# bjack205/LQR.jl

Measured on NVIDIA B200. Metric: batched LQR KKT solves/sec (FP64), higher is better.
Workload: dtype f64

## Files before the change

### lqr.jl_b200/csrc/riccati.cu

```cuda
#include <algorithm>
#include <cstdio>

#include "riccati_kernels.cuh"
#include "riccati_dmma_kernels.cuh"
#include "riccati_cta_kernels.cuh"

#define RICCATI_TPI_SIZES(X) \
    X(2, 1) X(3, 2) X(4, 1) X(4, 2) X(6, 3) X(2, 2) X(3, 1) X(3, 3) X(4, 3) X(5, 1) X(5, 2) X(5, 3) X(6, 1) X(6, 2)

static bool riccati_has_tpi(int n, int m) {
#define X(N_, M_) \
    if (n == N_ && m == M_) return true;
    RICCATI_TPI_SIZES(X)
#undef X
    return false;
}

#define RICCATI_DMMA_SIZES(X) X(8, 1) X(8, 2) X(8, 3) X(8, 4) X(12, 1) X(12, 2) X(12, 3) X(12, 4)

static bool riccati_has_dmma(int n, int m) {
#define X(N_, M_) \
    if (n == N_ && m == M_) return true;
    RICCATI_DMMA_SIZES(X)
#undef X
    return false;
}

#define RICCATI_CTA_SIZES(X) X(16, 8) X(16, 16) X(24, 8) X(24, 16) X(32, 8) X(32, 16) X(48, 16) X(64, 16)

static bool riccati_has_cta(int n, int m) {
#define X(N_, M_) \
    if (n == N_ && m == M_) return true;
    RICCATI_CTA_SIZES(X)
#undef X
    return false;
}

int lqrb_riccati_tile(const lqrb_context *h, int n, int m) {
    const int64_t force = h->opt("riccati_variant", 0);
    if (force == 2) return 1;
    return riccati_has_tpi(n, m) ? LQRB_TILE : 1;
}

static std::vector<RowMap> riccati_knot_map(int n, int m, int N, int flags) {
    const int Kn = (flags & LQRB_FLAG_LTI) ? 1 : N - 1;
    std::vector<RowMap> map;
    map.reserve((size_t)Kn * (n * n + n * m + tri(n) + tri(m) + n + m));
    for (int k = 0; k < Kn; ++k) {
        for (int e = 0; e < n * n; ++e) map.push_back({0, k * n * n + e, 0.0});
        for (int e = 0; e < n * m; ++e) map.push_back({1, k * n * m + e, 0.0});
        for (int j = 0; j < n; ++j)
            for (int i = 0; i <= j; ++i) map.push_back({2, k * n * n + i + j * n, 0.0});
        for (int j = 0; j < m; ++j)
            for (int i = 0; i <= j; ++i) map.push_back({3, k * m * m + i + j * m, 0.0});
        for (int e = 0; e < n; ++e) map.push_back({4, k * n + e, 0.0});
        for (int e = 0; e < m; ++e) map.push_back({5, k * m + e, 0.0});
        if (lqrb_riccati_knot_rows(n, m) > n * n + n * m + tri(n) + tri(m) + n + m) map.push_back({-1, 0, 0.0});
    }
    return map;
}

static std::vector<RowMap> riccati_term_map(int n) {
    std::vector<RowMap> map;
    for (int j = 0; j < n; ++j)
        for (int i = 0; i <= j; ++i) map.push_back({6, i + j * n, 0.0});
    for (int e = 0; e < n; ++e) map.push_back({7, e, 0.0});
    for (int e = 0; e < n; ++e) map.push_back({8, e, 0.0});
    return map;
}

static std::vector<RowMap> riccati_gain_map(int n, int m, int N) {
    std::vector<RowMap> map;
    for (int k = 0; k < N - 1; ++k) {
        for (int e = 0; e < m * n; ++e) map.push_back({0, k * m * n + e, 0.0});
        for (int e = 0; e < m; ++e) map.push_back({1, k * m + e, 0.0});
    }
    return map;
}

static std::string key(const char *tag, int a, int b, int c, int d) {
    char buf[96];
    snprintf(buf, sizeof buf, "%s:%d:%d:%d:%d", tag, a, b, c, d);
    return buf;
}

static int32_t check_dims(lqrb_context *h, int n, int m, int N, int64_t batch) {
    if (!h) return -1;
    if (n < 1 || n > 128) return lqrb_fail(h, -2, "n out of range [1,128]");
    if (m < 1 || m > n) return lqrb_fail(h, -3, "m out of range [1,n]");
    if (N < 2) return lqrb_fail(h, -4, "N must be >= 2");
    if (batch < 0) return lqrb_fail(h, -5, "batch must be >= 0");
    return 0;
}

template <int n, int m, bool LTI, int THREADS, int MINB>
static void launch_tpi_cfg(int N, int64_t batch, const double *knots, const double *term, double *Z,
                           double *gains, int32_t *info, cudaStream_t s) {
    const unsigned grid = (unsigned)((batch + THREADS - 1) / THREADS);
    riccati_tpi_kernel<n, m, LTI, THREADS, MINB><<<grid, THREADS, 0, s>>>(knots, term, Z, gains, info, N, batch);
}

template <int n, int m>
static int32_t launch_tpi(lqrb_context *h, int N, int64_t batch, int lti, const double *knots,
                          const double *term, double *Z, double *gains, int32_t *info,
                          cudaStream_t s) {
    constexpr bool SMALL = (n * n + n * m) <= 20;
    const bool tight = SMALL && h->opt("riccati_tpi_cfg", 0) != 1;
    if (SMALL && tight) {
        if (lti) launch_tpi_cfg<n, m, true, 64, 8>(N, batch, knots, term, Z, gains, info, s);
        else launch_tpi_cfg<n, m, false, 64, 8>(N, batch, knots, term, Z, gains, info, s);
    } else {
        if (lti) launch_tpi_cfg<n, m, true, 128, 1>(N, batch, knots, term, Z, gains, info, s);
        else launch_tpi_cfg<n, m, false, 128, 1>(N, batch, knots, term, Z, gains, info, s);
    }
    char nm[64];
    snprintf(nm, sizeof nm, "riccati_tpi<%d,%d>%s%s", n, m, lti ? "[lti]" : "", tight ? "[64x8]" : "[128x1]");
    h->kernel_name = nm;
    LQRB_LAUNCH_CHECK(h, "riccati_tpi_kernel");
    return 0;
}

static int32_t launch_coop(lqrb_context *h, int n, int m, int N, int64_t batch, int lti,
                           const double *knots, const double *term, double *Z, double *gains,
                           int32_t *info, cudaStream_t s) {
    const size_t per = riccati_coop_smem_doubles(n, m) * sizeof(double);
    char nm[64];
    if (n + m <= 24) {
        constexpr int G = 32, THREADS = 128;
        const size_t smem = per * (THREADS / G);
        auto kern = riccati_coop_kernel<G, THREADS>;
        LQRB_CUDA(h, cudaFuncSetAttribute(kern, cudaFuncAttributeMaxDynamicSharedMemorySize, (int)smem));
        const unsigned grid = (unsigned)((batch + THREADS / G - 1) / (THREADS / G));
        kern<<<grid, THREADS, smem, s>>>(knots, term, Z, gains, info, n, m, N, lti, batch);
        snprintf(nm, sizeof nm, "riccati_coop<G=32>(n=%d,m=%d)", n, m);
    } else {
        constexpr int G = 256, THREADS = 256;
        if (per > 227 * 1024) return lqrb_fail(h, -2, "n,m too large for the shared-memory Riccati kernel");
        auto kern = riccati_coop_kernel<G, THREADS>;
        LQRB_CUDA(h, cudaFuncSetAttribute(kern, cudaFuncAttributeMaxDynamicSharedMemorySize, (int)per));
        kern<<<(unsigned)batch, THREADS, per, s>>>(knots, term, Z, gains, info, n, m, N, lti, batch);
        snprintf(nm, sizeof nm, "riccati_coop<G=256>(n=%d,m=%d)", n, m);
    }
    h->kernel_name = nm;
    LQRB_LAUNCH_CHECK(h, "riccati_coop_kernel");
    return 0;
}

template <int n, int m>
static int32_t launch_dmma(lqrb_context *h, int N, int64_t batch, int lti, const double *knots,
                           const double *term, double *Z, double *gains, int32_t *info,
                           cudaStream_t s) {
    constexpr int STAGES = 3, WARPS = 4, MINB = m == 1 ? 6 : 5;
    const size_t smem = rdmma::riccati_dmma_warp_smem(rdmma::Map<n, m>::F, STAGES) * WARPS;
    auto kern = rdmma::riccati_dmma_kernel<n, m, STAGES, WARPS, MINB>;
    LQRB_CUDA(h, cudaFuncSetAttribute(kern, cudaFuncAttributeMaxDynamicSharedMemorySize, (int)smem));
    const unsigned grid = (unsigned)((batch + WARPS - 1) / WARPS);
    kern<<<grid, WARPS * 32, smem, s>>>(knots, term, Z, gains, info, N, lti, batch);
    char nm[64];
    snprintf(nm, sizeof nm, "riccati_dmma<%d,%d>%s", n, m, lti ? "[lti]" : "");
    h->kernel_name = nm;
    LQRB_LAUNCH_CHECK(h, "riccati_dmma_kernel");
    return 0;
}

template <int n, int m>
static int32_t launch_cta(lqrb_context *h, int N, int64_t batch, int lti, const double *knots,
                          const double *term, double *Z, double *gains, int32_t *info, cudaStream_t s) {
    using C = rcta::Cfg<n, m>;
    auto kern = rcta::riccati_cta_kernel<n, m>;
    LQRB_CUDA(h, cudaFuncSetAttribute(kern, cudaFuncAttributeMaxDynamicSharedMemorySize, (int)C::SMEM));
    kern<<<(unsigned)batch, C::THREADS, C::SMEM, s>>>(knots, term, Z, gains, info, N, lti, batch);
    char nm[64];
    snprintf(nm, sizeof nm, "riccati_cta_dmma<%d,%d>%s", n, m, lti ? "[lti]" : "");
    h->kernel_name = nm;
    LQRB_LAUNCH_CHECK(h, "riccati_cta_kernel");
    return 0;
}

static bool riccati_pad_target(const lqrb_context *h, int n, int m, int *n2, int *m2) {
    if (h->opt("riccati_pad", 1) == 0 || h->opt("riccati_variant", 0) != 0) return false;
    if (lqrb_riccati_tile(h, n, m) == LQRB_TILE || riccati_has_dmma(n, m) || riccati_has_cta(n, m)) return false;
#define X(N_, M_) \
    if (n <= N_ && m <= M_) { *n2 = N_; *m2 = M_; return true; }
    RICCATI_DMMA_SIZES(X)
    RICCATI_CTA_SIZES(X)
#undef X
    return false;
}

namespace {
struct RiccatiPadMaps {
    std::vector<RowMap> knots, term, z, gains;
};
}

static RiccatiPadMaps riccati_pad_maps(int n, int m, int N, int Kn, int n2, int m2) {
    RiccatiPadMaps M;
    const int F = lqrb_riccati_knot_rows(n, m), F2 = lqrb_riccati_knot_rows(n2, m2);
    const int nn = n * n, nm = n * m, tn = tri(n), tm = tri(m);
    for (int k = 0; k < Kn; ++k) {
        const int32_t b = k * F;
        const size_t start = M.knots.size();
        for (int j = 0; j < n2; ++j)
            for (int i = 0; i < n2; ++i) M.knots.push_back((i < n && j < n) ? RowMap{0, b + i + j * n, 0.0} : RowMap{-1, 0, 0.0});
        for (int j = 0; j < m2; ++j)
            for (int i = 0; i < n2; ++i)
                M.knots.push_back((i < n && j < m) ? RowMap{0, b + nn + i + j * n, 0.0} : RowMap{-1, 0, 0.0});
        for (int j = 0; j < n2; ++j)
            for (int i = 0; i <= j; ++i)
                M.knots.push_back(j < n ? RowMap{0, b + nn + nm + j * (j + 1) / 2 + i, 0.0} : RowMap{-1, 0, i == j ? 1.0 : 0.0});
        for (int j = 0; j < m2; ++j)
            for (int i = 0; i <= j; ++i)
                M.knots.push_back(j < m ? RowMap{0, b + nn + nm + tn + j * (j + 1) / 2 + i, 0.0} : RowMap{-1, 0, i == j ? 1.0 : 0.0});
        for (int i = 0; i < n2; ++i) M.knots.push_back(i < n ? RowMap{0, b + nn + nm + tn + tm + i, 0.0} : RowMap{-1, 0, 0.0});
        for (int i = 0; i < m2; ++i) M.knots.push_back(i < m ? RowMap{0, b + nn + nm + tn + tm + n + i, 0.0} : RowMap{-1, 0, 0.0});
        while (M.knots.size() - start < (size_t)F2) M.knots.push_back(RowMap{-1, 0, 0.0});
    }
    for (int j = 0; j < n2; ++j)
        for (int i = 0; i <= j; ++i) M.term.push_back(j < n ? RowMap{0, j * (j + 1) / 2 + i, 0.0} : RowMap{-1, 0, i == j ? 1.0 : 0.0});
    for (int i = 0; i < n2; ++i) M.term.push_back(i < n ? RowMap{0, tn + i, 0.0} : RowMap{-1, 0, 0.0});
    for (int i = 0; i < n2; ++i) M.term.push_back(i < n ? RowMap{0, tn + n + i, 0.0} : RowMap{-1, 0, 0.0});
    for (int k = 0; k < N; ++k) {
        for (int i = 0; i < n2; ++i) M.z.push_back(i < n ? RowMap{0, k * (n + m) + i, 0.0} : RowMap{-1, 0, 0.0});
        if (k < N - 1)
            for (int i = 0; i < m2; ++i) M.z.push_back(i < m ? RowMap{0, k * (n + m) + n + i, 0.0} : RowMap{-1, 0, 0.0});
    }
    const int GR = m * n + m;
    for (int k = 0; k < N - 1; ++k) {
        for (int j = 0; j < n2; ++j)
            for (int c = 0; c < m2; ++c) M.gains.push_back((c < m && j < n) ? RowMap{0, k * GR + c + m * j, 0.0} : RowMap{-1, 0, 0.0});
        for (int c = 0; c < m2; ++c) M.gains.push_back(c < m ? RowMap{0, k * GR + m * n + c, 0.0} : RowMap{-1, 0, 0.0});
    }
    return M;
}

static int32_t riccati_solve_on(lqrb_context *h, int n, int m, int N, int64_t batch, int flags, const double *knots,
                                const double *term, double *Z, double *gains, int32_t *info, Lane lane);

static int32_t riccati_solve_padded(lqrb_context *h, int n, int m, int N, int n2, int m2, int64_t batch, int flags,
                                    const double *knots, const double *term, double *Z, double *gains, int32_t *info,
                                    Lane lane) {
    const int Kn = (flags & LQRB_FLAG_LTI) ? 1 : N - 1;
    const int64_t F = lqrb_riccati_knot_rows(n, m), F2 = lqrb_riccati_knot_rows(n2, m2);
    const int64_t TR = tri(n) + 2 * n, TR2 = tri(n2) + 2 * n2;
    const int64_t ZR = (int64_t)N * n + (int64_t)(N - 1) * m, ZR2 = (int64_t)N * n2 + (int64_t)(N - 1) * m2;
    const int64_t GR = (int64_t)(N - 1) * (m * n + m), GR2 = (int64_t)(N - 1) * (m2 * n2 + m2);
    const std::string k0 = key("rpad", n, m, N, Kn) + key("->", n2, m2, 0, 0);
    DevMap mk, mt, mz, mg;
    if (h->maps.find(k0 + ":g") == h->maps.end()) {
        const RiccatiPadMaps M = riccati_pad_maps(n, m, N, Kn, n2, m2);
        mk = lqrb_get_map(h, k0 + ":k", M.knots);
        mt = lqrb_get_map(h, k0 + ":t", M.term);
        mz = lqrb_get_map(h, k0 + ":z", M.z);
        mg = lqrb_get_map(h, k0 + ":g", M.gains);
    } else {
        mk = h->maps[k0 + ":k"];
        mt = h->maps[k0 + ":t"];
        mz = h->maps[k0 + ":z"];
        mg = h->maps[k0 + ":g"];
    }
    if (mk.rows != Kn * F2 || mt.rows != TR2 || mz.rows != ZR2 || mg.rows != GR2) return lqrb_fail(h, 1, "pad map size mismatch");
    const int64_t per = Kn * F2 + TR2 + ZR2 + GR2;
    int64_t chunk = std::max<int64_t>(LQRB_TILE, ((int64_t)2 << 30) / (per * 8) / LQRB_TILE * LQRB_TILE);
    chunk = std::min(chunk, lqrb_padded_batch(batch));
    const size_t slice = ((size_t)chunk * per * 8 + 255) / 256 * 256;
    char *base = (char *)lqrb_scratch(h, SCR_RICCATI_PAD, slice, lane.index);
    if (!base) return 1000 + (int)cudaErrorMemoryAllocation;
    double *knots2 = (double *)base, *term2 = knots2 + chunk * Kn * F2, *Z2 = term2 + chunk * TR2, *gains2 = Z2 + chunk * ZR2;
    std::string name;
    for (int64_t first = 0; first < batch; first += chunk) {
        const int64_t cb = std::min(chunk, batch - first);
        ArrayTable src = {};
// ... 292 lines not shown
```

### lqr.jl_b200/csrc/riccati_dmma_kernels.cuh

```cuda
#pragma once
#include "smallmat.cuh"

namespace rdmma {

__device__ __forceinline__ void mma884(double &d0, double &d1, double a, double b) {
    asm("mma.sync.aligned.m8n8k4.row.col.f64.f64.f64.f64 {%0,%1}, {%2}, {%3}, {%0,%1};"
        : "+d"(d0), "+d"(d1)
        : "d"(a), "d"(b));
}

__device__ __forceinline__ uint32_t smem_u32(const void *p) { return (uint32_t)__cvta_generic_to_shared(p); }

__device__ __forceinline__ void mbar_init(uint64_t *bar, int count) {
    asm volatile("mbarrier.init.shared::cta.b64 [%0], %1;" ::"r"(smem_u32(bar)), "r"(count) : "memory");
}
__device__ __forceinline__ void mbar_expect_tx(uint64_t *bar, uint32_t bytes) {
    asm volatile("mbarrier.arrive.expect_tx.shared::cta.b64 _, [%0], %1;" ::"r"(smem_u32(bar)), "r"(bytes) : "memory");
}
__device__ __forceinline__ void mbar_wait(uint64_t *bar, uint32_t parity) {
    uint32_t ok = 0;
    const uint32_t a = smem_u32(bar);
    do {
        asm volatile(
            "{\n .reg .pred p;\n mbarrier.try_wait.parity.shared::cta.b64 p, [%1], %2;\n selp.u32 %0, 1, 0, p;\n}"
            : "=r"(ok)
            : "r"(a), "r"(parity)
            : "memory");
    } while (!ok);
}
__device__ __forceinline__ void bulk_g2s(void *dst, const void *src, uint32_t bytes, uint64_t *bar) {
    asm volatile("cp.async.bulk.shared::cluster.global.mbarrier::complete_tx::bytes [%0], [%1], %2, [%3];" ::"r"(
                     smem_u32(dst)),
                 "l"(src), "r"(bytes), "r"(smem_u32(bar))
                 : "memory");
}

template <int n, int m>
struct Map {
    static_assert(n == 8 || n == 12, "state tile map is written for n = 8, 12");
    static_assert(m >= 1 && m <= 4, "one control per quad lane");
    static constexpr int w = n + m;
    static constexpr int KS = n / 4;
    static constexpr int oQ = n * w, oR = oQ + tri(n), oq = oR + tri(m), orr = oq + n;
    static constexpr int F = lqrb_riccati_knot_rows(n, m);
    static constexpr int TR = tri(n) + 2 * n;
    static constexpr int GR = m * n + m;
    static_assert(F % 2 == 0, "bulk copies need 16-byte records");
    __host__ __device__ static constexpr int zmap(int pos) {
        if (pos < 8) return pos;
        const int j = pos - 8;
        if ((j & 1) == 0) return (8 + j / 2 < n) ? 8 + j / 2 : -1;
        return ((j - 1) / 2 < m) ? n + (j - 1) / 2 : -1;
    }
    __host__ __device__ static constexpr int xmap(int pos) {
        if (pos < 8) return pos;
        if (pos == 9) return -2;
        const int j = pos - 8;
        if ((j & 1) == 0) return (8 + j / 2 < n) ? 8 + j / 2 : -1;
        return -1;
    }
    __host__ __device__ static constexpr int kperm(int s, int q) { return s == 0 ? 2 * q : s == 1 ? 2 * q + 1 : 8 + q; }
};

#define RDMMA_AUX 184
__host__ __device__ inline size_t riccati_dmma_warp_smem(int F, int stages) {
    return ((size_t)stages * F * 8 + RDMMA_AUX * 8 + (size_t)stages * 8 + 15) / 16 * 16;
}

__device__ __forceinline__ double fast_rcp(double x) {
    double r;
    asm("rcp.approx.ftz.f64 %0, %1;" : "=d"(r) : "d"(x));
    double e = fma(-x, r, 1.0);
    r = fma(r, e, r);
    e = fma(-x, r, 1.0);
    return fma(r, e, r);
}

__device__ __forceinline__ double fast_rcp3(double x) {
    double r;
    asm("rcp.approx.ftz.f64 %0, %1;" : "=d"(r) : "d"(x));
    const double e = fma(-x, r, 1.0);
    const double t = fma(e, e, e);
    return fma(r, t, r);
}

template <int m>
__device__ __forceinline__ int spd_inv_row(double (&a)[4][4], int q, double (&mi)[4]) {
    int info = 0;
    double l[4][4], r[4];
    SM_UNROLL
    for (int j = 0; j < m; ++j) {
        if (info == 0 && !(a[j][j] > 0.0)) info = j + 1;
        r[j] = fast_rcp3(a[j][j]);
        SM_UNROLL
        for (int i = j + 1; i < m; ++i) l[i][j] = a[j][i] * r[j];
        SM_UNROLL
        for (int i = j + 1; i < m; ++i)
            SM_UNROLL
            for (int k = i; k < m; ++k) a[i][k] = fma(-l[i][j], a[j][k], a[i][k]);
    }
    SM_UNROLL
    for (int i = 0; i < m; ++i) {
        double s = q == i ? 1.0 : 0.0;
        SM_UNROLL
        for (int j = 0; j < i; ++j) s = fma(-l[i][j], mi[j], s);
        mi[i] = s;
    }
    SM_UNROLL
    for (int i = m - 1; i >= 0; --i) {
        double s = mi[i] * r[i];
        SM_UNROLL
        for (int j = i + 1; j < m; ++j) s = fma(-l[j][i], mi[j], s);
        mi[i] = s;
    }
    return info;
}

template <int n, int m, int STAGES, int WARPS, int MINB>
__global__ void __launch_bounds__(WARPS * 32, MINB)
    riccati_dmma_kernel(const double *__restrict__ knots, const double *__restrict__ term,
                        double *__restrict__ Z, double *__restrict__ gains, int32_t *__restrict__ info,
                        int N, int lti, int64_t batch) {
    using L = Map<n, m>;
    constexpr int F = L::F, KS = L::KS, w = L::w, GR = L::GR;
    constexpr bool HAS_X1 = n > 8;
    extern __shared__ __align__(16) unsigned char smem_raw[];
    const int warp = threadIdx.x >> 5, lane = threadIdx.x & 31;
    const int g = lane >> 2, q = lane & 3;
    const int64_t inst = (int64_t)blockIdx.x * WARPS + warp;
    if (inst >= batch) return;

    unsigned char *wbase = smem_raw + (size_t)warp * riccati_dmma_warp_smem(F, STAGES);
    double *buf = reinterpret_cast<double *>(wbase);
    double *aux = buf + (size_t)STAGES * F;
    uint64_t *full = reinterpret_cast<uint64_t *>(aux + RDMMA_AUX);
    double *V0d = aux, *Qd = aux + 64, *V1e = aux + 128, *gud = aux + 160, *G1e = aux + 168, *zero = aux + 172;
    double *zs = aux, *gs = aux + 32;

    if (lane == 0) {
        SM_UNROLL
        for (int s = 0; s < STAGES; ++s) mbar_init(full + s, 1);
        asm volatile("fence.mbarrier_init.release.cluster;" ::: "memory");
    }
    if (lane < 8) zero[lane] = 0.0;
    __syncwarp();

    const int Kn = lti ? 1 : N - 1;
    const double *rec_g = knots + inst * (int64_t)Kn * F;
    const double *tb = term + inst * L::TR;
    double *zb = Z + inst * ((int64_t)N * n + (int64_t)(N - 1) * m);
    double *gb = gains + inst * (int64_t)(N - 1) * GR;
    const int steps = N - 1;

    const bool odd = g & 1;
    const int su = (g - 1) >> 1;
    const int zc1 = odd ? (su < m ? n + su : -1) : (HAS_X1 && 8 + g / 2 < n ? 8 + g / 2 : -1);
    const double *pf0 = buf + 2 * q + n * g;
    const double *pf1 = buf + 2 * q + n * (zc1 >= 0 ? zc1 : 0);
    const bool has1 = zc1 >= 0;
    auto qoff = [](int i, int j) { return L::oQ + (i <= j ? j * (j + 1) / 2 + i : i * (i + 1) / 2 + j); };
    const double *ph00a = buf + qoff(g, 2 * q), *ph00b = buf + qoff(g, 2 * q + 1);
    const double *ph01 = buf + qoff(g, HAS_X1 ? 8 + q : 0);
    int o11 = L::oQ;
    bool v11 = false;
    if (!odd) {
        if (HAS_X1 && 8 + g / 2 < n) { o11 = qoff(8 + g / 2, 8 + q); v11 = true; }
    } else if (su < m && q < m) {
        o11 = L::oR + (su <= q ? q * (q + 1) / 2 + su : su * (su + 1) / 2 + q);
        v11 = true;
    }
    const double *ph11 = buf + o11;
    const double *pq0 = buf + L::oq + g;
    const double *pq1 = buf + (zc1 >= 0 ? (zc1 < n ? L::oq + zc1 : L::orr + (zc1 - n)) : L::oq);
    const int go0 = q < m ? q + m * g : -1;
    const int go1 = q < m ? (odd ? (g == 1 ? m * n + q : -1) : (HAS_X1 && 8 + g / 2 < n ? q + m * (8 + g / 2) : -1)) : -1;
    const double *rv0 = V0d + 8 * g;
    const double *rv1 = (!odd) ? V1e + 8 * (g >> 1) : ((g == 1 && q < m) ? gud : zero);
    const double *rt10 = g == 1 ? G1e + q : zero;
    const double hsel0 = g == 2 * q ? 0.5 : 0.0, hsel1 = g == 2 * q + 1 ? 0.5 : 0.0;

    double P[2][2][2];
    SM_UNROLL
    for (int rt = 0; rt < 2; ++rt)
        SM_UNROLL
        for (int ct = 0; ct < 2; ++ct)
            SM_UNROLL
            for (int e = 0; e < 2; ++e) {
// ... 201 lines not shown
```

### lqr.jl_b200/csrc/riccati_kernels.cuh

```cuda
#pragma once
#include "smallmat.cuh"

template <int n, int m>
struct RiccatiRows {
    static constexpr int oA = 0, oB = n * n, oQ = oB + n * m, oR = oQ + tri(n), oq = oR + tri(m),
                         orr = oq + n, F = lqrb_riccati_knot_rows(n, m);
    static constexpr int TR = tri(n) + 2 * n;
    static constexpr int GR = m * n + m;
    static constexpr int W = n + m;
};

template <int n, int m>
__device__ __forceinline__ int riccati_step(const double *A, const double *B, const double *Q,
                                            const double *R, const double *q, const double *r,
                                            double *P, double *p, double *K, double *kff) {
    double PB[n * m], PA[n * n], E[tri(m)], Einv[m], Kraw[m * n], rr[m];
    SM_UNROLL
    for (int j = 0; j < m; ++j)
        SM_UNROLL
        for (int i = 0; i < n; ++i) {
            double s = 0.0;
            SM_UNROLL
            for (int l = 0; l < n; ++l) s = fma(P[sym_idx(i, l)], B[l + j * n], s);
            PB[i + j * n] = s;
        }
    SM_UNROLL
    for (int j = 0; j < n; ++j)
        SM_UNROLL
        for (int i = 0; i < n; ++i) {
            double s = 0.0;
            SM_UNROLL
            for (int l = 0; l < n; ++l) s = fma(P[sym_idx(i, l)], A[l + j * n], s);
            PA[i + j * n] = s;
        }
    SM_UNROLL
    for (int j = 0; j < m; ++j)
        SM_UNROLL
        for (int i = 0; i <= j; ++i) {
            double s = R[tri_idx(i, j)];
            SM_UNROLL
            for (int l = 0; l < n; ++l) s = fma(B[l + i * n], PB[l + j * n], s);
            E[tri_idx(i, j)] = s;
        }
    SM_UNROLL
    for (int j = 0; j < n; ++j)
        SM_UNROLL
        for (int i = 0; i < m; ++i) {
            double s = 0.0;
            SM_UNROLL
            for (int l = 0; l < n; ++l) s = fma(B[l + i * n], PA[l + j * n], s);
            Kraw[i + j * m] = s;
            K[i + j * m] = s;
        }
    SM_UNROLL
    for (int i = 0; i < m; ++i) {
        double s = r[i];
        SM_UNROLL
        for (int l = 0; l < n; ++l) s = fma(B[l + i * n], p[l], s);
        rr[i] = s;
        kff[i] = s;
    }
    const int st = chol_packed<m>(E, Einv);
    SM_UNROLL
    for (int j = 0; j < n; ++j) solve_chol<m>(E, Einv, K + j * m);
    solve_chol<m>(E, Einv, kff);
    double pn[n];
    SM_UNROLL
    for (int i = 0; i < n; ++i) {
        double s = q[i];
        SM_UNROLL
        for (int l = 0; l < n; ++l) s = fma(A[l + i * n], p[l], s);
        SM_UNROLL
        for (int l = 0; l < m; ++l) s = fma(-K[l + i * m], rr[l], s);
        pn[i] = s;
    }
    SM_UNROLL
    for (int j = 0; j < n; ++j)
        SM_UNROLL
        for (int i = 0; i <= j; ++i) {
            double s = Q[tri_idx(i, j)];
            SM_UNROLL
            for (int l = 0; l < n; ++l) s = fma(A[l + i * n], PA[l + j * n], s);
            SM_UNROLL
            for (int l = 0; l < m; ++l) s = fma(-Kraw[l + i * m], K[l + j * m], s);
            P[tri_idx(i, j)] = s;
        }
    SM_UNROLL
    for (int i = 0; i < n; ++i) p[i] = pn[i];
    return st;
}

template <int n, int m, bool LTI, int THREADS, int MINB>
__global__ void __launch_bounds__(THREADS, MINB)
    riccati_tpi_kernel(const double *__restrict__ knots, const double *__restrict__ term,
                       double *__restrict__ Z, double *__restrict__ gains,
                       int32_t *__restrict__ info, int N, int64_t batch) {
    using L = RiccatiRows<n, m>;
    const int64_t inst = (int64_t)blockIdx.x * THREADS + threadIdx.x;
    if (inst >= batch) return;
    const int64_t tile = inst >> 5;
    const int lane = (int)(inst & 31);
    const int Kn = LTI ? 1 : N - 1;
    const double *kb = knots + tile * Kn * L::F * 32 + lane;
    const double *tb = term + tile * L::TR * 32 + lane;
    double *zb = Z + tile * ((int64_t)N * n + (int64_t)(N - 1) * m) * 32 + lane;
    double *gb = gains + tile * (int64_t)(N - 1) * L::GR * 32 + lane;

    double P[tri(n)], p[n];
    SM_UNROLL
    for (int e = 0; e < tri(n); ++e) P[e] = ld_stream(tb + e * 32);
    SM_UNROLL
    for (int e = 0; e < n; ++e) p[e] = ld_stream(tb + (tri(n) + e) * 32);

    double A[n * n], B[n * m];
    int st_all = 0;
    for (int k = N - 2; k >= 0; --k) {
        const double *kp = kb + (int64_t)(LTI ? 0 : k) * L::F * 32;
        double Q[tri(n)], R[tri(m)], q[n], r[m];
        SM_UNROLL
        for (int e = 0; e < n * n; ++e) A[e] = ld_keep(kp + (L::oA + e) * 32);
        SM_UNROLL
        for (int e = 0; e < n * m; ++e) B[e] = ld_keep(kp + (L::oB + e) * 32);
        SM_UNROLL
        for (int e = 0; e < tri(n); ++e) Q[e] = ld_stream(kp + (L::oQ + e) * 32);
        SM_UNROLL
        for (int e = 0; e < tri(m); ++e) R[e] = ld_stream(kp + (L::oR + e) * 32);
        SM_UNROLL
        for (int e = 0; e < n; ++e) q[e] = ld_stream(kp + (L::oq + e) * 32);
        SM_UNROLL
        for (int e = 0; e < m; ++e) r[e] = ld_stream(kp + (L::orr + e) * 32);
        double K[m * n], kff[m];
        const int st = riccati_step<n, m>(A, B, Q, R, q, r, P, p, K, kff);
        if (st != 0 && st_all == 0) st_all = (k + 1) * 1000 + st;
        double *gk = gb + (int64_t)k * L::GR * 32;
        SM_UNROLL
        for (int e = 0; e < m * n; ++e) gk[e * 32] = K[e];
        SM_UNROLL
        for (int e = 0; e < m; ++e) gk[(m * n + e) * 32] = kff[e];
    }
    if (info) info[inst] = st_all;

    double x[n];
    SM_UNROLL
    for (int e = 0; e < n; ++e) x[e] = ld_stream(tb + (tri(n) + n + e) * 32);
    for (int k = 0; k < N - 1; ++k) {
        const double *kp = kb + (int64_t)(LTI ? 0 : k) * L::F * 32;
        const double *gk = gb + (int64_t)k * L::GR * 32;
        double K[m * n], kff[m], u[m], xn[n];
        SM_UNROLL
        for (int e = 0; e < n * n; ++e) A[e] = ld_stream(kp + (L::oA + e) * 32);
        SM_UNROLL
        for (int e = 0; e < n * m; ++e) B[e] = ld_stream(kp + (L::oB + e) * 32);
        SM_UNROLL
        for (int e = 0; e < m * n; ++e) K[e] = gk[e * 32];
        SM_UNROLL
        for (int e = 0; e < m; ++e) kff[e] = gk[(m * n + e) * 32];
        double *zk = zb + (int64_t)k * L::W * 32;
        SM_UNROLL
        for (int i = 0; i < n; ++i) __stcs(zk + i * 32, x[i]);
        SM_UNROLL
        for (int i = 0; i < m; ++i) {
            double s = -kff[i];
            SM_UNROLL
            for (int l = 0; l < n; ++l) s = fma(-K[i + l * m], x[l], s);
            u[i] = s;
            __stcs(zk + (n + i) * 32, s);
        }
        SM_UNROLL
        for (int i = 0; i < n; ++i) {
            double s = 0.0;
            SM_UNROLL
            for (int l = 0; l < n; ++l) s = fma(A[i + l * n], x[l], s);
            SM_UNROLL
            for (int l = 0; l < m; ++l) s = fma(B[i + l * n], u[l], s);
            xn[i] = s;
        }
        SM_UNROLL
        for (int i = 0; i < n; ++i) x[i] = xn[i];
    }
    double *zN = zb + (int64_t)(N - 1) * L::W * 32;
    SM_UNROLL
    for (int i = 0; i < n; ++i) __stcs(zN + i * 32, x[i]);
}

template <int G>
__device__ __forceinline__ void group_sync() {
    if (G <= 32)
        __syncwarp();
    else
        __syncthreads();
}

__host__ __device__ inline size_t riccati_coop_smem_doubles(int n, int m) {
    return (size_t)4 * n * n + 4 * n * m + m * m + 4 * n + 3 * m + 8;
}

template <int G, int THREADS>
__global__ void __launch_bounds__(THREADS)
    riccati_coop_kernel(const double *__restrict__ knots, const double *__restrict__ term,
                        double *__restrict__ Z, double *__restrict__ gains,
                        int32_t *__restrict__ info, int n, int m, int N, int lti, int64_t batch) {
    extern __shared__ double smem[];
    constexpr int IPC = THREADS / G;
    const int g = threadIdx.x / G, t = threadIdx.x % G;
    const int64_t inst_raw = (int64_t)blockIdx.x * IPC + g;
    const bool active = inst_raw < batch;
    const int64_t inst = active ? inst_raw : batch - 1;
    const int nn = n * n, nm = n * m, tn = tri(n), tm = tri(m);
    const int F = lqrb_riccati_knot_rows(n, m), TR = tn + 2 * n, GR = m * n + m, W = n + m;
    const int Kn = lti ? 1 : N - 1;
    double *s = smem + (size_t)g * riccati_coop_smem_doubles(n, m);
    double *P = s, *Pn = P + nn, *PA = Pn + nn, *A = PA + nn, *B = A + nn, *PB = B + nm,
           *Kraw = PB + nm, *K = Kraw + nm, *E = K + nm, *p = E + m * m, *pn = p + n, *x = pn + n,
           *xn = x + n, *rr = xn + n, *kff = rr + m, *u = kff + m;
    const double *rec = knots + inst * (int64_t)Kn * F;
    const double *tb = term + inst * TR;
    double *zb = Z + inst * ((int64_t)N * n + (int64_t)(N - 1) * m);
    double *gb = gains + inst * (int64_t)(N - 1) * GR;
    int st_all = 0;

    for (int e = t; e < nn; e += G) {
        const int i = e % n, j = e / n;
        P[e] = tb[sym_idx(i, j)];
    }
    for (int e = t; e < n; e += G) p[e] = tb[tn + e];
    group_sync<G>();

    for (int k = N - 2; k >= 0; --k) {
        const double *kp = rec + (int64_t)(lti ? 0 : k) * F;
        const double *Qp = kp + nn + nm, *Rp = Qp + tn, *qp = Rp + tm, *rp = qp + n;
        for (int e = t; e < nn; e += G) A[e] = kp[e];
        for (int e = t; e < nm; e += G) B[e] = kp[nn + e];
        group_sync<G>();
        for (int e = t; e < nn + nm; e += G) {
            const bool isA = e < nn;
            const int ee = isA ? e : e - nn;
            const int i = ee % n, j = ee / n;
            const double *col = (isA ? A : B) + j * n;
            double acc = 0.0;
            for (int l = 0; l < n; ++l) acc = fma(P[i + l * n], col[l], acc);
            (isA ? PA : PB)[ee] = acc;
        }
        group_sync<G>();
        for (int e = t; e < m * m + nm + m; e += G) {
            if (e < m * m) {
                const int i = e % m, j = e / m;
                double acc = Rp[sym_idx(i, j)];
                for (int l = 0; l < n; ++l) acc = fma(B[l + i * n], PB[l + j * n], acc);
                E[e] = acc;
            } else if (e < m * m + nm) {
                const int ee = e - m * m, i = ee % m, j = ee / m;
                double acc = 0.0;
                for (int l = 0; l < n; ++l) acc = fma(B[l + i * n], PA[l + j * n], acc);
                Kraw[ee] = acc;
                K[ee] = acc;
            } else {
                const int i = e - m * m - nm;
                double acc = rp[i];
                for (int l = 0; l < n; ++l) acc = fma(B[l + i * n], p[l], acc);
                rr[i] = acc;
                kff[i] = acc;
            }
        }
        group_sync<G>();
        for (int j = 0; j < m; ++j) {
            const double djj = E[j + j * m];
            if (!(djj > 0.0) && st_all == 0) st_all = (k + 1) * 1000 + j + 1;
            const double d = sqrt(djj);
            group_sync<G>();
            for (int i = j + t; i < m; i += G) E[j + i * m] = (i == j) ? d : E[j + i * m] / d;
            group_sync<G>();
            const int rem = m - j - 1;
            for (int e = t; e < rem * rem; e += G) {
                const int a = j + 1 + e % rem, b = j + 1 + e / rem;
                if (a <= b) E[a + b * m] = fma(-E[j + a * m], E[j + b * m], E[a + b * m]);
            }
            group_sync<G>();
        }
        for (int c = t; c < n + 1; c += G) {
            double *col = (c < n) ? K + c * m : kff;
            for (int i = 0; i < m; ++i) {
                double acc = col[i];
                for (int l = 0; l < i; ++l) acc = fma(-E[l + i * m], col[l], acc);
                col[i] = acc / E[i + i * m];
            }
            for (int i = m - 1; i >= 0; --i) {
                double acc = col[i];
                for (int l = i + 1; l < m; ++l) acc = fma(-E[i + l * m], col[l], acc);
                col[i] = acc / E[i + i * m];
            }
        }
        group_sync<G>();
        for (int e = t; e < nn + n; e += G) {
            if (e < nn) {
                const int i = e % n, j = e / n;
                double acc = Qp[sym_idx(i, j)];
                for (int l = 0; l < n; ++l) acc = fma(A[l + i * n], PA[l + j * n], acc);
                for (int l = 0; l < m; ++l) acc = fma(-Kraw[l + i * m], K[l + j * m], acc);
                Pn[e] = acc;
            } else {
                const int i = e - nn;
                double acc = qp[i];
                for (int l = 0; l < n; ++l) acc = fma(A[l + i * n], p[l], acc);
                for (int l = 0; l < m; ++l) acc = fma(-K[l + i * m], rr[l], acc);
                pn[i] = acc;
            }
        }
        if (active) {
            double *gk = gb + (int64_t)k * GR;
            for (int e = t; e < nm; e += G) gk[e] = K[e];
            for (int e = t; e < m; e += G) gk[nm + e] = kff[e];
        }
        group_sync<G>();
        for (int e = t; e < nn; e += G) {
            const int i = e % n, j = e / n;
            P[e] = (i <= j) ? Pn[e] : Pn[j + i * n];
        }
        for (int e = t; e < n; e += G) p[e] = pn[e];
        group_sync<G>();
    }
    if (active && info && t == 0) info[inst] = st_all;

    for (int e = t; e < n; e += G) x[e] = tb[tn + n + e];
    group_sync<G>();
    for (int k = 0; k < N - 1; ++k) {
        const double *kp = rec + (int64_t)(lti ? 0 : k) * F;
        const double *Ag = kp, *Bg = kp + nn;
        const double *gk = gb + (int64_t)k * GR;
        double *zk = zb + (int64_t)k * W;
        for (int i = t; i < m; i += G) {
            double acc = -gk[nm + i];
            for (int l = 0; l < n; ++l) acc = fma(-gk[i + l * m], x[l], acc);
            u[i] = acc;
        }
        group_sync<G>();
// ... 20 lines not shown
```

Measured before the change: 116.3 million.

## Stage TPI Riccati knots through TMA bulk-copy ring with L2 cache hints

Adds a persistent one-warp-per-tile TPI kernel. It streams per-knot records into a three-stage shared-memory ring using cp.async.bulk and mbarriers, instead of having each thread load directly from global memory. The grid size is chosen so that the working set of A/B and the gains stays within an L2 budget. A/B and gains are tagged evict_last so the forward pass can reread them from L2, and the rest is tagged evict_first. The cost is one-warp blocks with occupancy limited by the dynamic shared memory, serialised tile loops, and an extra misalignment fix-up path. This may reduce latency hiding compared with the old 64/128-thread direct-load kernel.

```diff
diff --git a/lqr.jl_b200/csrc/riccati.cu b/lqr.jl_b200/csrc/riccati.cu
--- a/lqr.jl_b200/csrc/riccati.cu
+++ b/lqr.jl_b200/csrc/riccati.cu
@@ -93,31 +93,60 @@
     return 0;
 }
 
-template <int n, int m, bool LTI, int THREADS, int MINB>
-static void launch_tpi_cfg(int N, int64_t batch, const double *knots, const double *term, double *Z,
-                           double *gains, int32_t *info, cudaStream_t s) {
-    const unsigned grid = (unsigned)((batch + THREADS - 1) / THREADS);
-    riccati_tpi_kernel<n, m, LTI, THREADS, MINB><<<grid, THREADS, 0, s>>>(knots, term, Z, gains, info, N, batch);
+#define RICCATI_TPI_MIN_WARPS 4
+#define RICCATI_TPI_L2_BUDGET ((int64_t)96 << 20)
+
+template <int n, int m>
+constexpr bool riccati_tpi_staged() {
+    return RICCATI_TPI_MIN_WARPS * (TpiRing<n, m, false>::BYTES + 1024) <= 228 * 1024;
+}
+
+template <int n, int m, bool LTI>
+static int32_t launch_tpi_tiles(lqrb_context *h, int N, int64_t batch, const double *knots, const double *term,
+                                double *Z, double *gains, int32_t *info, cudaStream_t s) {
+    using RG = TpiRing<n, m, LTI>;
+    auto kern = riccati_tpi_tiles_kernel<n, m, LTI>;
+    LQRB_CUDA(h, cudaFuncSetAttribute(kern, cudaFuncAttributeMaxDynamicSharedMemorySize, (int)RG::BYTES));
+    int per_sm = 0;
+    LQRB_CUDA(h, cudaOccupancyMaxActiveBlocksPerMultiprocessor(&per_sm, kern, 32, RG::BYTES));
+    const int64_t tiles = (batch + LQRB_TILE - 1) / LQRB_TILE, resident = std::max<int64_t>(1, (int64_t)per_sm * h->sm_count);
+    const int64_t keep = ((int64_t)(LTI ? 1 : N - 1) * (n * n + n * m) + (int64_t)(N - 1) * (m * n + m)) * 256;
+    const int64_t force = h->opt("riccati_tpi_tiles", 0);
+    int64_t inflight;
+    if (force > 0) {
+        inflight = std::min({force, resident, tiles});
+    } else {
+        const int64_t fit = RICCATI_TPI_L2_BUDGET / std::max<int64_t>(1, keep / 2);
+        inflight = std::min({std::max<int64_t>(fit, (int64_t)RICCATI_TPI_MIN_WARPS * h->sm_count), resident, tiles});
+        const int64_t rounds = (tiles + inflight - 1) / inflight;
+        inflight = (tiles + rounds - 1) / rounds;
+    }
+    kern<<<(unsigned)inflight, 32, RG::BYTES, s>>>(knots, term, Z, gains, info, N, batch);
+    char nm[80];
+    snprintf(nm, sizeof nm, "riccati_tpi<%d,%d>%s[%lld tiles]", n, m, LTI ? "[lti]" : "", (long long)inflight);
+    h->kernel_name = nm;
+    LQRB_LAUNCH_CHECK(h, "riccati_tpi_tiles_kernel");
+    return 0;
 }
 
 template <int n, int m>
 static int32_t launch_tpi(lqrb_context *h, int N, int64_t batch, int lti, const double *knots,
                           const double *term, double *Z, double *gains, int32_t *info,
                           cudaStream_t s) {
-    constexpr bool SMALL = (n * n + n * m) <= 20;
-    const bool tight = SMALL && h->opt("riccati_tpi_cfg", 0) != 1;
-    if (SMALL && tight) {
-        if (lti) launch_tpi_cfg<n, m, true, 64, 8>(N, batch, knots, term, Z, gains, info, s);
-        else launch_tpi_cfg<n, m, false, 64, 8>(N, batch, knots, term, Z, gains, info, s);
+    if constexpr (riccati_tpi_staged<n, m>()) {
+        return lti ? launch_tpi_tiles<n, m, true>(h, N, batch, knots, term, Z, gains, info, s)
+                   : launch_tpi_tiles<n, m, false>(h, N, batch, knots, term, Z, gains, info, s);
     } else {
-        if (lti) launch_tpi_cfg<n, m, true, 128, 1>(N, batch, knots, term, Z, gains, info, s);
-        else launch_tpi_cfg<n, m, false, 128, 1>(N, batch, knots, term, Z, gains, info, s);
-    }
-    char nm[64];
-    snprintf(nm, sizeof nm, "riccati_tpi<%d,%d>%s%s", n, m, lti ? "[lti]" : "", tight ? "[64x8]" : "[128x1]");
-    h->kernel_name = nm;
-    LQRB_LAUNCH_CHECK(h, "riccati_tpi_kernel");
-    return 0;
+        constexpr int THREADS = 128;
+        const unsigned grid = (unsigned)((batch + THREADS - 1) / THREADS);
+        if (lti) riccati_tpi_kernel<n, m, true, THREADS, 1><<<grid, THREADS, 0, s>>>(knots, term, Z, gains, info, N, batch);
+        else riccati_tpi_kernel<n, m, false, THREADS, 1><<<grid, THREADS, 0, s>>>(knots, term, Z, gains, info, N, batch);
+        char nm[64];
+        snprintf(nm, sizeof nm, "riccati_tpi<%d,%d>%s[128x1]", n, m, lti ? "[lti]" : "");
+        h->kernel_name = nm;
+        LQRB_LAUNCH_CHECK(h, "riccati_tpi_kernel");
+        return 0;
+    }
 }
 
 static int32_t launch_coop(lqrb_context *h, int n, int m, int N, int64_t batch, int lti,
diff --git a/lqr.jl_b200/csrc/riccati_dmma_kernels.cuh b/lqr.jl_b200/csrc/riccati_dmma_kernels.cuh
--- a/lqr.jl_b200/csrc/riccati_dmma_kernels.cuh
+++ b/lqr.jl_b200/csrc/riccati_dmma_kernels.cuh
@@ -33,6 +33,26 @@
                      smem_u32(dst)),
                  "l"(src), "r"(bytes), "r"(smem_u32(bar))
                  : "memory");
+}
+__device__ __forceinline__ void bulk_g2s_hint(void *dst, const void *src, uint32_t bytes, uint64_t *bar, uint64_t pol) {
+    asm volatile(
+        "cp.async.bulk.shared::cluster.global.mbarrier::complete_tx::bytes.L2::cache_hint [%0], [%1], %2, [%3], %4;" ::"r"(
+            smem_u32(dst)),
+        "l"(src), "r"(bytes), "r"(smem_u32(bar)), "l"(pol)
+        : "memory");
+}
+__device__ __forceinline__ uint64_t l2_evict_last() {
+    uint64_t p;
+    asm volatile("createpolicy.fractional.L2::evict_last.b64 %0, 1.0;" : "=l"(p));
+    return p;
+}
+__device__ __forceinline__ uint64_t l2_evict_first() {
+    uint64_t p;
+    asm volatile("createpolicy.fractional.L2::evict_first.b64 %0, 1.0;" : "=l"(p));
+    return p;
+}
+__device__ __forceinline__ void st_hint(double *p, double v, uint64_t pol) {
+    asm volatile("st.global.L2::cache_hint.f64 [%0], %1, %2;" ::"l"(p), "d"(v), "l"(pol) : "memory");
 }
 
 template <int n, int m>
diff --git a/lqr.jl_b200/csrc/riccati_kernels.cuh b/lqr.jl_b200/csrc/riccati_kernels.cuh
--- a/lqr.jl_b200/csrc/riccati_kernels.cuh
+++ b/lqr.jl_b200/csrc/riccati_kernels.cuh
@@ -1,5 +1,6 @@
 #pragma once
 #include "smallmat.cuh"
+#include "riccati_dmma_kernels.cuh"
 
 template <int n, int m>
 struct RiccatiRows {
@@ -181,6 +182,203 @@
     double *zN = zb + (int64_t)(N - 1) * L::W * 32;
     SM_UNROLL
     for (int i = 0; i < n; ++i) __stcs(zN + i * 32, x[i]);
+}
+
+template <int n, int m, bool LTI>
+struct TpiRing {
+    using L = RiccatiRows<n, m>;
+    static constexpr int STAGES = 3;
+    static constexpr int AB = n * n + n * m;
+    static constexpr int REC = L::F * 32 + 2;
+    static constexpr int GAIN = L::GR * 32 + 2;
+    static constexpr int FWD = AB * 32 + 2 + GAIN;
+    static constexpr int STG = LTI ? GAIN : (REC > FWD ? REC : FWD);
+    static constexpr int DOUBLES = STAGES * STG + (LTI ? REC : 0);
+    static constexpr size_t BYTES = (size_t)DOUBLES * 8 + (STAGES + 1) * 8;
+};
+
+template <int n, int m, bool LTI>
+__global__ void __launch_bounds__(32, 1)
+    riccati_tpi_tiles_kernel(const double *__restrict__ knots, const double *__restrict__ term,
+                             double *__restrict__ Z, double *__restrict__ gains,
+                             int32_t *__restrict__ info, int N, int64_t batch) {
+    using L = RiccatiRows<n, m>;
+    using RG = TpiRing<n, m, LTI>;
+    constexpr int S = RG::STAGES, AB = RG::AB, F = L::F, GR = L::GR;
+    extern __shared__ __align__(16) unsigned char smem_raw[];
+    double *ring = reinterpret_cast<double *>(smem_raw);
+    double *lrec = ring + S * RG::STG;
+    uint64_t *bar = reinterpret_cast<uint64_t *>(ring + RG::DOUBLES);
+    const int lane = threadIdx.x;
+    if (lane == 0) {
+        SM_UNROLL
+        for (int s = 0; s <= S; ++s) rdmma::mbar_init(bar + s, 1);
+        asm volatile("fence.mbarrier_init.release.cluster;" ::: "memory");
+    }
+    __syncwarp();
+    const uint64_t keep = rdmma::l2_evict_last(), drop = rdmma::l2_evict_first();
+    const int Kn = LTI ? 1 : N - 1, steps = N - 1;
+    const int64_t tiles = (batch + 31) >> 5;
+    const int ks = (int)(((uintptr_t)knots >> 3) & 1), gsh = (int)(((uintptr_t)gains >> 3) & 1);
+    uint32_t issued = 0, used = 0, lti_par = 0;
+
+    auto fill_last = [&](double *dst, const double *chunk, int doubles) {
+        if (lane == 31) {
+            dst[doubles] = chunk[doubles - 1];
+            asm volatile("fence.proxy.async.shared::cta;" ::: "memory");
+        }
+    };
+
+    for (int64_t tile = blockIdx.x; tile < tiles; tile += gridDim.x) {
+        const int64_t inst = tile * 32 + lane;
+        const bool active = inst < batch;
+        const double *kb = knots + tile * Kn * F * 32;
+        double *gb = gains + tile * (int64_t)steps * GR * 32;
+        const double *tb = term + tile * L::TR * 32 + lane;
+        double *zb = Z + tile * ((int64_t)N * n + (int64_t)(N - 1) * m) * 32 + lane;
+
+        auto issue_bwd = [&](int k) {
+            double *dst = ring + (issued % S) * RG::STG;
+            const double *src = kb + (int64_t)k * F * 32;
+            if (lane == 0) {
+                uint64_t *b = bar + issued % S;
+                rdmma::mbar_expect_tx(b, F * 256);
+                rdmma::bulk_g2s_hint(dst, src - ks, AB * 256, b, keep);
+                rdmma::bulk_g2s_hint(dst + AB * 32, src - ks + AB * 32, (F - AB) * 256, b, drop);
+            }
+            if (ks) fill_last(dst, src, F * 32);
+            ++issued;
+        };
+        auto issue_fwd = [&](int k) {
+            double *dst = ring + (issued % S) * RG::STG;
+            double *gdst = LTI ? dst : dst + AB * 32 + 2;
+            const double *gsrc = gb + (int64_t)k * GR * 32;
+            if (lane == 0) {
+                uint64_t *b = bar + issued % S;
+                const uint32_t ab = LTI ? 0 : AB * 256 + (ks ? 16 : 0);
+                rdmma::mbar_expect_tx(b, ab + GR * 256);
+                if (!LTI) rdmma::bulk_g2s_hint(dst, kb + (int64_t)k * F * 32 - ks, ab, b, drop);
+                rdmma::bulk_g2s_hint(gdst, gsrc - gsh, GR * 256, b, drop);
+            }
+            if (gsh) fill_last(gdst, gsrc, GR * 32);
+            ++issued;
+        };
+        auto wait = [&]() -> double * {
+            const uint32_t c = used++;
+            rdmma::mbar_wait(bar + c % S, (c / S) & 1);
+            return ring + (c % S) * RG::STG;
+        };
+
+        __syncwarp();
+        if (LTI) {
+            if (lane == 0) {
+                rdmma::mbar_expect_tx(bar + S, F * 256);
+                rdmma::bulk_g2s_hint(lrec, kb - ks, F * 256, bar + S, keep);
+            }
+            if (ks) fill_last(lrec, kb, F * 32);
+        } else {
+            for (int j = 0; j < S - 1 && j < steps; ++j) issue_bwd(steps - 1 - j);
+        }
+
+        double P[tri(n)], p[n];
+        SM_UNROLL
+        for (int e = 0; e < tri(n); ++e) P[e] = ld_stream(tb + e * 32);
+        SM_UNROLL
+        for (int e = 0; e < n; ++e) p[e] = ld_stream(tb + (tri(n) + e) * 32);
+        if (LTI) {
+            rdmma::mbar_wait(bar + S, lti_par);
+            lti_par ^= 1;
+        }
+
+        double A[n * n], B[n * m];
+        int st_all = 0;
+        for (int k = steps - 1; k >= 0; --k) {
+            const double *kp;
+            if (LTI) {
+                kp = lrec + ks + lane;
+            } else {
+                __syncwarp();
+                if (k - (S - 1) >= 0) issue_bwd(k - (S - 1));
+                kp = wait() + ks + lane;
+            }
+            double Q[tri(n)], R[tri(m)], q[n], r[m];
+            SM_UNROLL
+            for (int e = 0; e < n * n; ++e) A[e] = kp[(L::oA + e) * 32];
+            SM_UNROLL
+            for (int e = 0; e < n * m; ++e) B[e] = kp[(L::oB + e) * 32];
+            SM_UNROLL
+            for (int e = 0; e < tri(n); ++e) Q[e] = kp[(L::oQ + e) * 32];
+            SM_UNROLL
+            for (int e = 0; e < tri(m); ++e) R[e] = kp[(L::oR + e) * 32];
+            SM_UNROLL
+            for (int e = 0; e < n; ++e) q[e] = kp[(L::oq + e) * 32];
+            SM_UNROLL
+            for (int e = 0; e < m; ++e) r[e] = kp[(L::orr + e) * 32];
+            double K[m * n], kff[m];
+            const int st = riccati_step<n, m>(A, B, Q, R, q, r, P, p, K, kff);
+            if (st != 0 && st_all == 0) st_all = (k + 1) * 1000 + st;
+            if (active) {
+                double *gk = gb + (int64_t)k * GR * 32 + lane;
+                SM_UNROLL
+                for (int e = 0; e < m * n; ++e) rdmma::st_hint(gk + e * 32, K[e], keep);
+                SM_UNROLL
+                for (int e = 0; e < m; ++e) rdmma::st_hint(gk + (m * n + e) * 32, kff[e], keep);
+            }
+        }
+        if (active && info) info[inst] = st_all;
+
+        asm volatile("fence.proxy.async.global;" ::: "memory");
+        __syncwarp();
+        for (int j = 0; j < S - 1 && j < steps; ++j) issue_fwd(j);
+        double x[n];
+        SM_UNROLL
+        for (int e = 0; e < n; ++e) x[e] = ld_stream(tb + (tri(n) + n + e) * 32);
+        for (int k = 0; k < steps; ++k) {
+            __syncwarp();
+            if (k + S - 1 < steps) issue_fwd(k + S - 1);
+            const double *stg = wait();
+            const double *kp = (LTI ? lrec : stg) + ks + lane;
+            const double *gk = (LTI ? stg : stg + AB * 32 + 2) + gsh + lane;
+            double K[m * n], kff[m], u[m], xn[n];
+            SM_UNROLL
+            for (int e = 0; e < n * n; ++e) A[e] = kp[(L::oA + e) * 32];
+            SM_UNROLL
+            for (int e = 0; e < n * m; ++e) B[e] = kp[(L::oB + e) * 32];
+            SM_UNROLL
+            for (int e = 0; e < m * n; ++e) K[e] = gk[e * 32];
+            SM_UNROLL
+            for (int e = 0; e < m; ++e) kff[e] = gk[(m * n + e) * 32];
+            double *zk = zb + (int64_t)k * L::W * 32;
+            if (active) {
+                SM_UNROLL
+                for (int i = 0; i < n; ++i) __stcs(zk + i * 32, x[i]);
+            }
+            SM_UNROLL
+            for (int i = 0; i < m; ++i) {
+                double s = -kff[i];
+                SM_UNROLL
+                for (int l = 0; l < n; ++l) s = fma(-K[i + l * m], x[l], s);
+                u[i] = s;
+                if (active) __stcs(zk + (n + i) * 32, s);
+            }
+            SM_UNROLL
+            for (int i = 0; i < n; ++i) {
+                double s = 0.0;
+                SM_UNROLL
+                for (int l = 0; l < n; ++l) s = fma(A[i + l * n], x[l], s);
+                SM_UNROLL
+                for (int l = 0; l < m; ++l) s = fma(B[i + l * n], u[l], s);
+                xn[i] = s;
+            }
+            SM_UNROLL
+            for (int i = 0; i < n; ++i) x[i] = xn[i];
+        }
+        if (active) {
+            double *zN = zb + (int64_t)(N - 1) * L::W * 32;
+            SM_UNROLL
+            for (int i = 0; i < n; ++i) __stcs(zN + i * 32, x[i]);
+        }
+    }
 }
 
 template <int G>
```

Result: faster. 125.9 million (median of 6 runs) (+8.3%).
